# lavajuno/afskmodem

Measured on AMD Instinct MI355X. Metric: Msamples/s demodulated (batched 48 kHz streams) + decoded-byte match rate vs CPU ref, higher is better.
Workload: dtype int16

## Files before the change

### afskmodem_amd/batch.py

```python
from __future__ import annotations

import ctypes as C
import threading
import math
import os
from dataclasses import dataclass

import numpy as np

from . import _native

SAMPLE_RATE = _native.SAMPLE_RATE
SYNC_WINDOW = _native.SYNC_WINDOW


def validate_bit_frames(bit_frames) -> None:
    bf = np.atleast_1d(np.asarray(bit_frames))
    if np.any(bf <= 0) or np.any(SAMPLE_RATE % np.maximum(bf, 1) != 0) or np.any(bf % 2 != 0):
        raise Exception("Invalid baud rate.")
    if np.any(2 * bf >= SYNC_WINDOW):
        raise IndexError("list index out of range")
    if np.any(bf % 4 != 0):
        raise Exception("Comparing two waveforms of different lengths.")


_I32_MAX, _I32_MIN = 2 ** 31 - 1, -2 ** 31


def threshold_lt(t) -> int:
    t = float(t)
    if math.isnan(t):
        return _I32_MIN
    if math.isinf(t):
        return _I32_MAX if t > 0 else _I32_MIN
    return max(_I32_MIN, min(_I32_MAX, math.ceil(t)))


def threshold_gt(t) -> int:
    t = float(t)
    if math.isnan(t):
        return _I32_MAX
    if math.isinf(t):
        return _I32_MAX if t > 0 else _I32_MIN
    return max(_I32_MIN, min(_I32_MAX, math.floor(t)))


def out_stride_for(max_len: int, min_bit_frames: int) -> int:
    s = int(max_len // (14 * max(min_bit_frames, 4)) + 2 + 3) & ~3
    return s if s <= 192 else (s + 127) & ~127




@dataclass
class HostDemodResult:
    bytes: np.ndarray
    nbytes: np.ndarray
    nbits: np.ndarray
    clock_idx: np.ndarray
    term_frame: np.ndarray
    status: np.ndarray

    def payloads(self) -> list[bytes]:
        stride = self.bytes.shape[1]
        return [self.bytes[i, : min(int(n), stride)].tobytes() for i, n in enumerate(self.nbytes)]


def demod_host_arrays(arrays, bit_frames, amp_end_threshold: int = 14000) -> HostDemodResult:
    n = len(arrays)
    keep = [np.ascontiguousarray(a, dtype=np.int16).reshape(-1) for a in arrays]
    lens = np.array([a.size for a in keep], dtype=np.int32)
    bf = np.broadcast_to(np.asarray(bit_frames, dtype=np.int32), (n,)).copy()
    if n:
        validate_bit_frames(bf)
    stride = out_stride_for(int(lens.max()) if n else 0, int(bf.min()) if n else 4)
    res = HostDemodResult(np.zeros((n, stride), np.uint8), *(np.zeros(n, np.int32) for _ in range(5)))
    if n == 0:
        return res
    if n == 1:
        return demod_host_flat(keep[0], [0], lens, bf, amp_end_threshold, stride)
    ptrs = (C.c_void_p * n)(*[a.__array_interface__["data"][0] for a in keep])
    p = lambda a, t: a.ctypes.data_as(C.POINTER(t))
    _native.check(_native.lib().afsk_demod_streams_host(
        ptrs, p(lens, C.c_int32), p(bf, C.c_int32), threshold_lt(amp_end_threshold), n,
        p(res.bytes, C.c_uint8), stride, p(res.nbytes, C.c_int32), p(res.nbits, C.c_int32),
        p(res.clock_idx, C.c_int32), p(res.term_frame, C.c_int32), p(res.status, C.c_int32)))
    return res


def demod_host_flat(flat, stream_offset, stream_len, bit_frames,
                    amp_end_threshold: int = 14000, out_stride: int | None = None) -> HostDemodResult:
    flat = np.ascontiguousarray(flat, dtype=np.int16).reshape(-1)
    offs = np.ascontiguousarray(stream_offset, dtype=np.int64)
    lens = np.ascontiguousarray(stream_len, dtype=np.int32)
    n = offs.size
    bf = np.broadcast_to(np.asarray(bit_frames, dtype=np.int32), (n,)).copy()
    if n:
        validate_bit_frames(bf)
    stride = out_stride if out_stride is not None else out_stride_for(
        int(lens.max()) if n else 0, int(bf.min()) if n else 4)
    res = HostDemodResult(np.zeros((n, stride), np.uint8), *(np.zeros(n, np.int32) for _ in range(5)))
    if n == 0:
        return res
    total = flat.size
    if total == 0:
        flat = np.zeros(1, np.int16)
    p = lambda a, t: a.ctypes.data_as(C.POINTER(t))
    _native.check(_native.lib().afsk_demod_batch_host(
        p(flat, C.c_int16), total, p(offs, C.c_int64), p(lens, C.c_int32), p(bf, C.c_int32),
        threshold_lt(amp_end_threshold), n, p(res.bytes, C.c_uint8), stride, p(res.nbytes, C.c_int32),
        p(res.nbits, C.c_int32), p(res.clock_idx, C.c_int32), p(res.term_frame, C.c_int32),
        p(res.status, C.c_int32)))
    return res




def _torch():
    import torch
    return torch


@dataclass
class DemodResult:
    bytes: "object"
    nbytes: "object"
    nbits: "object"
    clock_idx: "object"
    term_frame: "object"
    status: "object"
    corrected: "object" = None
    margins: "object" = None

    def symbols_demodulated(self, bit_frames) -> "object":
        torch = _torch()
        bf = torch.as_tensor(bit_frames, device=self.nbits.device).to(torch.int64)
        found = (self.term_frame.to(torch.int64) - self.clock_idx.to(torch.int64)) // bf \
            + self.nbits.to(torch.int64)
        return found

    def cpu(self) -> HostDemodResult:
        return HostDemodResult(*(t.cpu().numpy() for t in
                                 (self.bytes, self.nbytes, self.nbits, self.clock_idx,
                                  self.term_frame, self.status)))

    def payloads(self) -> list[bytes]:
        return self.cpu().payloads()


def flat_layout(n_streams: int, out_stride: int):
    nb = (n_streams * out_stride + 3) & ~3
    offs = [0] + [nb + 4 * n_streams * k for k in range(5)]
    return offs, nb + 20 * n_streams


def views_of_flat(flat, n_streams: int, out_stride: int) -> "DemodResult":
    torch = _torch()
    offs, total = flat_layout(n_streams, out_stride)
    assert flat.numel() == total and flat.dtype == torch.uint8
    i32 = [flat[o: o + 4 * n_streams].view(torch.int32) for o in offs[1:]]
    res = DemodResult(flat[: n_streams * out_stride].view(n_streams, out_stride), *i32)
    res.flat = flat
    return res


def alloc_result(n_streams: int, out_stride: int, device) -> DemodResult:
    torch = _torch()
    _, total = flat_layout(n_streams, out_stride)
    return views_of_flat(torch.zeros(total, dtype=torch.uint8, device=device), n_streams, out_stride)


def uniform_layout(n_streams: int, stream_len: int, device):
    torch = _torch()
    off = torch.arange(n_streams, dtype=torch.int64, device=device) * int(stream_len)
    ln = torch.full((n_streams,), int(stream_len), dtype=torch.int32, device=device)
    return off, ln


def _as_device_i32(x, n, device):
    torch = _torch()
    if isinstance(x, torch.Tensor):
        return x.to(device=device, dtype=torch.int32).contiguous()
    arr = np.broadcast_to(np.asarray(x, dtype=np.int32), (n,)).copy()
    return torch.from_numpy(arr).to(device)


def _stream_ptr(stream, device=None):
    torch = _torch()
    s = stream if stream is not None else torch.cuda.current_stream(device)
    return C.c_void_p(s.cuda_stream)


def _same_device(dev, **tensors) -> None:
    for name, t in tensors.items():
        if t is not None and t.device != dev:
            raise ValueError(f"{name} is on {t.device}, samples on {dev}: all tensors of a launch must share one device")


def _order_after_current(stream, device) -> None:
    torch = _torch()
    if stream is not None:
        cur = torch.cuda.current_stream(device)
        if stream.cuda_stream != cur.cuda_stream:
            stream.wait_stream(cur)


def _uniform_bit_frames(bit_frames, n: int):
    if isinstance(bit_frames, (int, np.integer)):
        return int(bit_frames)
    if isinstance(bit_frames, (list, tuple, np.ndarray)):
        arr = np.asarray(bit_frames)
        if arr.ndim == 0:
            return int(arr)
        if arr.size not in (1, n):
            raise ValueError(f"bit_frames holds {arr.size} values for {n} streams (1 or {n} expected)")
        if arr.size and np.all(arr == arr.flat[0]):
            return int(arr.flat[0])
    return None


_PLAN_CACHE: "dict[tuple, GroupPlan]" = {}
_PLAN_CACHE_MAX = 8
_PLAN_CACHE_LOCK = threading.Lock()


def lengths_ragged(stream_len_host) -> bool:
    if stream_len_host is None:
        return False
    a = np.asarray(stream_len_host)
    return bool(a.size >= 8 and int(a.max()) > 0 and int(a.min()) * 4 < int(a.max()) * 3)


def _cached_plan(bit_frames, n: int, dev, stream_len_host=None) -> "GroupPlan":
    arr = np.asarray(bit_frames, dtype=np.int32)
    if arr.size not in (1, n):
        raise ValueError(f"bit_frames holds {arr.size} values for {n} streams (1 or {n} expected)")
    arr = np.ascontiguousarray(np.broadcast_to(arr.reshape(-1) if arr.ndim else arr, (n,)))
    lens = None
    if lengths_ragged(stream_len_host):
        lens = np.ascontiguousarray(np.asarray(stream_len_host, dtype=np.int32).reshape(-1))
        if lens.size != n:
            raise ValueError(f"stream_len_host holds {lens.size} values for {n} streams")
    key = (str(dev), n, hash(arr.tobytes()), None if lens is None else hash(lens.tobytes()))
    with _PLAN_CACHE_LOCK:
        plan = _PLAN_CACHE.pop(key, None)
        if plan is not None and np.array_equal(plan.bit_frames, arr) and (
                lens is None if plan.stream_len is None else (lens is not None and np.array_equal(plan.stream_len, lens))):
            _PLAN_CACHE[key] = plan
            return plan
    fresh = GroupPlan(arr, dev, stream_len=lens)
    with _PLAN_CACHE_LOCK:
        _PLAN_CACHE[key] = fresh
        while len(_PLAN_CACHE) > _PLAN_CACHE_MAX:
            _PLAN_CACHE.pop(next(iter(_PLAN_CACHE)))
    return fresh


class _NativePlan:
    _destroy: str

    def __init__(self, device):
        _native.require_device()
        _drain_parked_plans()
        self.device = _default_device(device)
        self._h = C.c_void_p()

    @property
    def handle(self):
        if not self._h:
            raise ValueError("the plan has been closed")
        return self._h

    def close(self) -> None:
        if self._h:
            getattr(_native.lib(), self._destroy)(self._h)
            self._h = C.c_void_p()

    def __del__(self):
        h = getattr(self, "_h", None)
        if not h:
            return
        self._h = None
        try:
            torch = _torch()
            if torch.cuda.is_current_stream_capturing():
                raise RuntimeError("capturing")
            torch.cuda.synchronize(self.device)
            getattr(_native.lib(), self._destroy)(h)
        except Exception:
            try:
                with _PARKED_LOCK:
                    _PARKED_PLANS.append((h, self.device, self._destroy))
            except Exception:
                pass


class GroupPlan(_NativePlan):
    _destroy = "afsk_group_plan_destroy"

    def __init__(self, bit_frames, device=None, stream_len=None):
        torch = _torch()
        super().__init__(device)
        self.bit_frames = np.ascontiguousarray(np.asarray(bit_frames, dtype=np.int32).reshape(-1))
        self.n = int(self.bit_frames.size)
        self.stream_len = None
        if stream_len is not None:
            self.stream_len = np.ascontiguousarray(np.asarray(stream_len, dtype=np.int32).reshape(-1))
            if self.stream_len.size != self.n:
                raise ValueError(f"stream_len holds {self.stream_len.size} values for {self.n} streams")
        i32 = C.POINTER(C.c_int32)
        with torch.cuda.device(self.device):
            _native.check(_native.lib().afsk_group_plan_create_ragged(
                self.bit_frames.ctypes.data_as(i32),
                None if self.stream_len is None else self.stream_len.ctypes.data_as(i32), self.n, C.byref(self._h)))

    def groups(self) -> list[tuple[int, int]]:
        ng, nn = C.c_int32(), C.c_int32()
        lib = _native.lib()
        _native.check(lib.afsk_group_plan_info(self.handle, C.byref(nn), C.byref(ng), None, None, 0))
        bf, cnt = (C.c_int32 * max(ng.value, 1))(), (C.c_int32 * max(ng.value, 1))()
        _native.check(lib.afsk_group_plan_info(self.handle, None, None, bf, cnt, ng.value))
        return [(int(bf[k]), int(cnt[k])) for k in range(ng.value)]


_PARKED_PLANS: list = []
_PARKED_LOCK = threading.Lock()


def _drain_parked_plans() -> None:
    if not _PARKED_PLANS:
        return
    torch = _torch()
    try:
        if torch.cuda.is_current_stream_capturing():
            return
    except Exception:
        return
    with _PARKED_LOCK:
        todo, _PARKED_PLANS[:] = list(_PARKED_PLANS), []
    for h, dev, destroy in todo:
        try:
            torch.cuda.synchronize(dev)
            getattr(_native.lib(), destroy)(h)
        except Exception:
            with _PARKED_LOCK:
                _PARKED_PLANS.append((h, dev, destroy))


def release_parked_plans() -> int:
    _drain_parked_plans()
    return len(_PARKED_PLANS)


def _check_index_tensors(dev, stream_offset, stream_len) -> None:
    torch = _torch()
    if stream_offset.dtype != torch.int64 or stream_len.dtype != torch.int32:
        raise TypeError("stream_offset must be int64 and stream_len int32")
    if not (stream_offset.is_cuda and stream_len.is_cuda):
        raise TypeError("stream_offset / stream_len must be CUDA tensors")
    _same_device(dev, stream_offset=stream_offset, stream_len=stream_len)
    if not (stream_offset.is_contiguous() and stream_len.is_contiguous()):
        raise ValueError("stream_offset / stream_len must be contiguous (the kernel reads them as plain arrays)")


def _prepare_outputs(out, out_stride, n: int, dev, diagnostics: bool, margin_stride):
    torch = _torch()
    fresh = False
    if out is None:
        if out_stride is None:
            raise ValueError("pass out= or out_stride=")
        out = alloc_result(n, int(out_stride), dev)
        fresh = True
    soft = (None, None, 0)
    if diagnostics:
        if out.corrected is None:
            out.corrected = torch.zeros(n, dtype=torch.int32, device=dev)
            fresh = True
        if out.margins is None:
            if margin_stride is None:
                raise ValueError("diagnostics=True needs margin_stride= (symbols per margins row)")
            out.margins = torch.zeros((n, int(margin_stride)), dtype=torch.int32, device=dev)
            fresh = True
        soft = (out.corrected.data_ptr(), out.margins.data_ptr(), int(out.margins.shape[1]))
    _same_device(dev, out_bytes=out.bytes, out_nbytes=out.nbytes, out_status=out.status)
    return out, fresh, (out.bytes.data_ptr(), int(out.bytes.shape[1]), out.nbytes.data_ptr(), out.nbits.data_ptr(),
                        out.clock_idx.data_ptr(), out.term_frame.data_ptr(), out.status.data_ptr(), *soft)


def demod_batch(samples, stream_offset, stream_len, bit_frames, amp_end_threshold: int = 14000,
                out: DemodResult | None = None, out_stride: int | None = None, stream=None,
                validate: bool = True, diagnostics: bool = False,
                margin_stride: int | None = None, entry: str = "auto", plan: "GroupPlan | None" = None,
                stream_len_host=None) -> DemodResult:
    torch = _torch()
    _native.require_device()
    if not (isinstance(samples, torch.Tensor) and samples.is_cuda and samples.dtype == torch.int16):
        raise TypeError("samples must be an int16 CUDA tensor (HBM resident)")
    if not samples.is_contiguous():
        raise ValueError("samples must be contiguous")
    if entry not in ("auto", "uniform", "grouped", "mixed"):
        raise ValueError("entry must be 'auto', 'uniform', 'grouped' or 'mixed'")
    n = int(stream_offset.numel())
    dev = samples.device
    if bit_frames is None and plan is None:
        raise ValueError("bit_frames=None needs plan= (the plan holds the batch's bit_frames)")
    if validate and bit_frames is not None and not isinstance(bit_frames, torch.Tensor):
        validate_bit_frames(bit_frames)
    _check_index_tensors(dev, stream_offset, stream_len)
    host_bf = isinstance(bit_frames, (int, np.integer, list, tuple, np.ndarray))
    if plan is not None:
        if entry not in ("auto", "grouped"):
            raise ValueError("plan= goes with entry='auto' or 'grouped'")
        if plan.n != n or plan.device != dev:
            raise ValueError(f"the plan covers {plan.n} streams on {plan.device}, the batch {n} on {dev}")
        entry = "grouped"
    ragged = plan is None and host_bf and entry in ("auto", "grouped") and lengths_ragged(stream_len_host)
    ubf = None if (entry in ("mixed", "grouped") or ragged) else _uniform_bit_frames(bit_frames, n)
    if entry == "uniform" and ubf is None:
        raise ValueError("entry='uniform' needs ONE bit_frames value (an int or an all-equal host sequence)")
    if entry == "grouped" and plan is None and not host_bf:
        raise ValueError("entry='grouped' needs host-side bit_frames (or plan=): a device tensor is never inspected")
    grouped = entry == "grouped" or ragged or (entry == "auto" and ubf is None and host_bf)
    out, fresh, outs = _prepare_outputs(out, out_stride, n, dev, diagnostics, margin_stride)
    amp = threshold_lt(amp_end_threshold)
    lib = _native.lib()
    with torch.cuda.device(dev):
        if fresh:
            _order_after_current(stream, dev)
        if ubf is not None:
            _native.check(lib.afsk_demod_batch_uniform(
                samples.data_ptr(), stream_offset.data_ptr(), stream_len.data_ptr(), ubf, amp, n, *outs,
                _stream_ptr(stream, dev)))
            return out
        if grouped:
            if plan is None:
                plan = _cached_plan(bit_frames, n, dev, stream_len_host if ragged else None)
            _native.check(lib.afsk_demod_batch_grouped(
                plan.handle, samples.data_ptr(), stream_offset.data_ptr(), stream_len.data_ptr(), amp, *outs,
                _stream_ptr(stream, dev)))
            out._plan_keepalive = plan
            return out
        bf = _as_device_i32(bit_frames, n, dev)
        _order_after_current(stream, dev)
        _native.check(lib.afsk_demod_batch_ex(
            samples.data_ptr(), stream_offset.data_ptr(), stream_len.data_ptr(), bf.data_ptr(), amp, n, *outs,
            _stream_ptr(stream, dev)))
    out._bf_keepalive = bf
    return out


VALID_BIT_FRAMES = tuple(bf for bf in range(4, SYNC_WINDOW // 2, 4) if SAMPLE_RATE % bf == 0)
assert len(VALID_BIT_FRAMES) == _native.DETECT_MAX_CANDIDATES


@dataclass
class HostRateResult:
    bit_frames: np.ndarray
    score: np.ndarray
    runner_up: np.ndarray
    clock_idx: np.ndarray
    scores: "np.ndarray | None"
    candidates: tuple

    def bauds(self) -> list:
        return [SAMPLE_RATE // int(bf) if bf > 0 else None for bf in self.bit_frames]


@dataclass
class RateResult:
    bit_frames: "object"
    score: "object"
    runner_up: "object"
    clock_idx: "object"
    scores: "object" = None
    candidates: tuple = ()

    def cpu(self) -> HostRateResult:
        h = lambda t: None if t is None else t.cpu().numpy()
        return HostRateResult(h(self.bit_frames), h(self.score), h(self.runner_up), h(self.clock_idx), h(self.scores),
                              self.candidates)

    def bauds(self) -> list:
        return self.cpu().bauds()


def check_candidates(candidates) -> tuple:
    if candidates is None:
        return VALID_BIT_FRAMES
    cands = tuple(int(c) for c in np.asarray(candidates).reshape(-1).tolist())
    if not 1 <= len(cands) <= _native.DETECT_MAX_CANDIDATES:
        raise ValueError(f"{len(cands)} candidates (1 ... {_native.DETECT_MAX_CANDIDATES} expected)")
    validate_bit_frames(cands)
    return cands


def detect_rates(samples, stream_offset, stream_len, candidates=None, out: RateResult | None = None, stream=None,
                 scores: bool = False) -> RateResult:
    torch = _torch()
    cands = check_candidates(candidates)
    _native.require_device()
    if not (isinstance(samples, torch.Tensor) and samples.is_cuda and samples.dtype == torch.int16):
        raise TypeError("samples must be an int16 CUDA tensor (HBM resident)")
    if not samples.is_contiguous():
        raise ValueError("samples must be contiguous")
    n = int(stream_offset.numel())
    dev = samples.device
    _check_index_tensors(dev, stream_offset, stream_len)
    if int(stream_len.numel()) != n:
        raise ValueError(f"{n} stream offsets for {int(stream_len.numel())} stream lengths")
    fresh = out is None
    if out is None:
        i32 = lambda *shape: torch.zeros(shape, dtype=torch.int32, device=dev)
        out = RateResult(i32(n), i32(n), i32(n), i32(n), i32(n, len(cands)) if scores else None, cands)
    else:
        want = {"bit_frames": (n,), "score": (n,), "runner_up": (n,), "clock_idx": (n,)}
        if scores or out.scores is not None:
            want["scores"] = (n, len(cands))
        for name, shape in want.items():
            t = getattr(out, name)
            if not (isinstance(t, torch.Tensor) and t.dtype == torch.int32 and tuple(t.shape) == shape
                    and t.is_contiguous()):
                raise ValueError(f"out.{name} must be a contiguous int32 tensor of shape {shape}")
        _same_device(dev, **{"out_" + name: getattr(out, name) for name in want})
        out.candidates = cands
    c_arr = (C.c_int32 * len(cands))(*cands)
    with torch.cuda.device(dev):
        if fresh:
            _order_after_current(stream, dev)
        _native.check(_native.lib().afsk_detect_rate_batch(
            samples.data_ptr(), stream_offset.data_ptr(), stream_len.data_ptr(), n, c_arr, len(cands),
            out.bit_frames.data_ptr(), out.score.data_ptr(), out.runner_up.data_ptr(), out.clock_idx.data_ptr(),
            None if out.scores is None else out.scores.data_ptr(), _stream_ptr(stream, dev)))
    return out


def _split_host_arrays(stream_len_host, bit_frames, segment_symbols):
    lens = np.ascontiguousarray(np.asarray(stream_len_host, dtype=np.int64).reshape(-1))
    n = int(lens.size)
    if n and (int(lens.min()) < 0 or int(lens.max()) > _native.MAX_STREAM_LEN):
        raise ValueError(f"stream lengths must lie in 0 ... {_native.MAX_STREAM_LEN}")
    bf = np.asarray(bit_frames)
    if bf.size not in (1, n) and not (n == 0 and bf.size == 0):
        raise ValueError(f"bit_frames holds {bf.size} values for {n} streams (1 or {n} expected)")
    bf = np.ascontiguousarray(np.broadcast_to(bf.reshape(-1) if bf.ndim else bf, (n,)).astype(np.int32))
    if n:
        validate_bit_frames(bf)
    segment_symbols = int(segment_symbols)
    if segment_symbols < 0 or segment_symbols % 64:
        raise ValueError("segment_symbols must be a multiple of 64 (0 = the default)")
    return lens.astype(np.int32), bf, segment_symbols


def split_scratch_bytes(stream_len_host, bit_frames, segment_symbols: int = 0) -> tuple[int, int]:
    lens, bf, seg = _split_host_arrays(stream_len_host, bit_frames, segment_symbols)
    i32 = C.POINTER(C.c_int32)
    nbytes, nseg = C.c_int64(), C.c_int32()
    _native.check(_native.lib().afsk_split_scratch_bytes(lens.ctypes.data_as(i32), bf.ctypes.data_as(i32), int(lens.size),
                                                         seg, C.byref(nbytes), C.byref(nseg)))
    return int(nbytes.value), int(nseg.value)


class SplitPlan(_NativePlan):
    _destroy = "afsk_split_plan_destroy"

    def __init__(self, stream_len_host, bit_frames, device=None, segment_symbols: int = 0):
        torch = _torch()
        lens, bf, seg = _split_host_arrays(stream_len_host, bit_frames, segment_symbols)
        super().__init__(device)
        self.stream_len = lens
        self.bit_frames = bf
        self.n = int(lens.size)
        self.segment_symbols = seg
        i32 = C.POINTER(C.c_int32)
        lib = _native.lib()
        with torch.cuda.device(self.device):
            _native.check(lib.afsk_split_plan_create(lens.ctypes.data_as(i32), bf.ctypes.data_as(i32), self.n, seg,
                                                     C.byref(self._h)))
            nseg, nbytes = C.c_int32(), C.c_int64()
            _native.check(lib.afsk_split_plan_info(self._h, None, C.byref(nseg), C.byref(nbytes)))
            self.n_segments = int(nseg.value)
            self.scratch_bytes = int(nbytes.value)
            self.scratch = torch.empty(max(self.scratch_bytes, 1), dtype=torch.uint8, device=self.device)


def demod_batch_split(samples, stream_offset, stream_len, plan: SplitPlan, amp_end_threshold: int = 14000,
                      out: DemodResult | None = None, out_stride: int | None = None, stream=None,
                      diagnostics: bool = False, margin_stride: int | None = None) -> DemodResult:
    torch = _torch()
    if not isinstance(plan, SplitPlan):
        raise TypeError("plan must be a SplitPlan")
    if not (isinstance(samples, torch.Tensor) and samples.dtype == torch.int16):
        raise TypeError("samples must be an int16 CUDA tensor (HBM resident)")
    if not (isinstance(stream_offset, torch.Tensor) and isinstance(stream_len, torch.Tensor)):
        raise TypeError("stream_offset / stream_len must be CUDA tensors")
    if stream_offset.dtype != torch.int64 or stream_len.dtype != torch.int32:
        raise TypeError("stream_offset must be int64 and stream_len int32")
    n = int(stream_offset.numel())
    if plan.n != n or int(stream_len.numel()) != n:
        raise ValueError(f"the plan covers {plan.n} streams, the batch {n}")
    if out is None and out_stride is None:
        raise ValueError("pass out= or out_stride=")
    if diagnostics and (out is None or out.margins is None) and margin_stride is None:
        raise ValueError("diagnostics=True needs margin_stride= (symbols per margins row)")
    _native.require_device()
    if not samples.is_cuda:
        raise TypeError("samples must be an int16 CUDA tensor (HBM resident)")
    if not samples.is_contiguous():
        raise ValueError("samples must be contiguous")
    dev = samples.device
    _check_index_tensors(dev, stream_offset, stream_len)
    if plan.device != dev:
        raise ValueError(f"the plan was built on {plan.device}, the batch lives on {dev}")
    out, fresh, outs = _prepare_outputs(out, out_stride, n, dev, diagnostics, margin_stride)
    with torch.cuda.device(dev):
        if fresh:
            _order_after_current(stream, dev)
        _native.check(_native.lib().afsk_demod_batch_split(
            plan.handle, samples.data_ptr(), stream_offset.data_ptr(), stream_len.data_ptr(),
            threshold_lt(amp_end_threshold), plan.scratch.data_ptr(), *outs, _stream_ptr(stream, dev)))
    out._plan_keepalive = plan
    return out


@dataclass
class GateResult:
    n_bursts: "object"
    burst_start: "object"
    burst_len: "object"
    open_end: "object"
    block_amp: "object"
    slot_offset: "object" = None
    slot_len: "object" = None

    def burst_streams(self, stream_offset):
        torch = _torch()
        nb = self.burst_start.shape[1]
        mask = torch.arange(nb, device=self.n_bursts.device)[None, :] < self.n_bursts[:, None]
        owner, k = torch.nonzero(mask, as_tuple=True)
        off = stream_offset[owner] + self.burst_start[owner, k].to(torch.int64)
        return owner, off.contiguous(), self.burst_len[owner, k].contiguous()

    def burst_slots(self, stream_offset):
        if self.slot_len is not None:
            return self.slot_offset.reshape(-1), self.slot_len.reshape(-1)
        torch = _torch()
        nb = self.burst_start.shape[1]
        mask = torch.arange(nb, device=self.n_bursts.device)[None, :] < self.n_bursts[:, None]
        off = torch.where(mask, stream_offset[:, None] + self.burst_start.to(torch.int64), 0)
        ln = torch.where(mask, self.burst_len, 0)
        return off.reshape(-1).contiguous(), ln.reshape(-1).contiguous()


def gate_batch(samples, stream_offset, stream_len, max_stream_len: int,
               amp_start_threshold: int = 18000, amp_end_threshold: int = 14000,
               max_bursts: int = 16, stream=None, slots: bool = True) -> GateResult:
    torch = _torch()
    _native.require_device()
    if not (isinstance(samples, torch.Tensor) and samples.is_cuda and samples.dtype == torch.int16
            and samples.is_contiguous()):
        raise TypeError("samples must be a contiguous int16 CUDA tensor")
    if stream_offset.dtype != torch.int64 or stream_len.dtype != torch.int32:
        raise TypeError("stream_offset must be int64 and stream_len int32")
    n = int(stream_offset.numel())
    dev = samples.device
    _same_device(dev, stream_offset=stream_offset, stream_len=stream_len)
    max_blocks = int(max_stream_len) // 2048
    i32 = lambda *shape: torch.zeros(shape, dtype=torch.int32, device=dev)
    with torch.cuda.device(dev):
        res = GateResult(i32(n), i32(n, max(max_bursts, 1)), i32(n, max(max_bursts, 1)), i32(n),
                         i32(n, max(max_blocks, 1)))
        if slots and max_bursts > 0:
            res.slot_offset = torch.zeros((n, int(max_bursts)), dtype=torch.int64, device=dev)
            res.slot_len = i32(n, int(max_bursts))
        _order_after_current(stream, dev)
        args = (samples.data_ptr(), stream_offset.data_ptr(), stream_len.data_ptr(), int(max_stream_len),
                threshold_gt(amp_start_threshold), threshold_lt(amp_end_threshold), n, int(max_bursts),
                res.block_amp.data_ptr(), res.n_bursts.data_ptr(), res.burst_start.data_ptr(),
                res.burst_len.data_ptr(), res.open_end.data_ptr())
        if res.slot_len is not None:
            _native.check(_native.lib().afsk_gate_batch_slots(*args, res.slot_offset.data_ptr(), res.slot_len.data_ptr(),
                                                              _stream_ptr(stream, dev)))
        else:
            _native.check(_native.lib().afsk_gate_batch(*args, _stream_ptr(stream, dev)))
    return res


def _default_device(device):
    torch = _torch()
    return torch.device("cuda", torch.cuda.current_device()) if device is None else torch.device(device)


def upload_streams(arrays, device=None):
    torch = _torch()
    _native.require_device()
    device = _default_device(device)
    lens = np.array([len(a) for a in arrays], dtype=np.int32)
    offs = np.zeros(len(arrays), dtype=np.int64)
    if len(arrays) > 1:
        offs[1:] = np.cumsum(lens[:-1], dtype=np.int64)
    flat = (np.concatenate([np.ascontiguousarray(a, dtype=np.int16) for a in arrays])
            if len(arrays) else np.zeros(0, np.int16))
    if flat.size == 0:
        flat = np.zeros(1, np.int16)
    t = lambda a: torch.from_numpy(a).to(device)
    return t(flat), t(offs), t(lens), int(lens.max()) if len(arrays) else 0


def read_wav_frames(filename: str) -> np.ndarray:
    import wave
    with wave.open(filename, "rb") as f:
        raw = f.readframes(f.getnframes())
    return np.frombuffer(raw, dtype="<i2", count=len(raw) // 2)


def _c_names(filenames):
    import sys
    strs = [f if type(f) is str else os.fsdecode(os.fspath(f)) for f in filenames]
    if not strs:
        return (b"", None), (C.c_char_p * 0)()
    blob = ("\0".join(strs) + "\0").encode(sys.getfilesystemencoding(), sys.getfilesystemencodeerrors())
    a = np.frombuffer(blob, np.uint8)
    ends = np.flatnonzero(a == 0)
    if ends.size != len(strs):
        raise ValueError("embedded null byte")
    ptrs = np.empty(len(strs), np.uint64)
    ptrs[0] = 0
    ptrs[1:] = ends[:-1] + 1
    ptrs += np.uint64(a.ctypes.data)
    return (blob, ptrs), C.cast(ptrs.ctypes.data, C.POINTER(C.c_char_p))


def _wav_probe_c(arr, n):
    off = np.zeros(n, np.int64)
    nbytes = np.zeros(n, np.int64)
    status = np.zeros(n, np.int32)
    if n:
        p = lambda a, t: a.ctypes.data_as(C.POINTER(t))
        _native.check(_native.lib().afsk_wav_probe(arr, n, p(off, C.c_int64), p(nbytes, C.c_int64),
                                                   p(status, C.c_int32)))
    return off, nbytes, status


def wav_probe(filenames):
    names = list(filenames)
    keep, arr = _c_names(names)
    res = _wav_probe_c(arr, len(names))
    del keep
    return res


def load_wav_batch(filenames, device=None):
    torch = _torch()
    _native.require_device()
    device = _default_device(device)
    names = list(filenames)
    if not names:
        return upload_streams([], device)
    n = len(names)
    enc, arr = _c_names(names)
    lib = _native.lib()
    p64 = lambda a: a.ctypes.data_as(C.POINTER(C.c_int64))
    sizes = np.zeros(n, np.int64)
    _native.check(lib.afsk_file_sizes(arr, n, p64(sizes)))
    slot = np.minimum(((np.maximum(sizes, 0) // 2) + 7) & ~np.int64(7), np.int64(_native.MAX_STREAM_LEN & ~7))
    offs = np.zeros(n, np.int64)
    offs[1:] = np.cumsum(slot[:-1])
    total = int(offs[-1] + slot[-1])
    samples = torch.empty(max(total, 1), dtype=torch.int16, device=device)
    if total == 0:
        samples.zero_()
    d_off = np.zeros(n, np.int64)
    d_bytes = np.zeros(n, np.int64)
    status = np.zeros(n, np.int32)
    torch.cuda.current_stream(samples.device).synchronize()
    with torch.cuda.device(samples.device):
        _native.check(lib.afsk_wav_ingest(arr, n, p64(offs), p64(slot), samples.data_ptr(), int(samples.numel()),
                                          p64(d_off), p64(d_bytes), status.ctypes.data_as(C.POINTER(C.c_int32))))
    lens = (d_bytes // 2).astype(np.int64)
    bad = np.nonzero(status != _native.WAV_OK)[0]
    if bad.size:
        lens[bad] = 0
        late = []
        for i in bad:
            fr = read_wav_frames(names[int(i)])
            lens[i] = len(fr)
            if len(fr) <= int(slot[i]):
                if len(fr):
                    samples[int(offs[i]): int(offs[i]) + len(fr)] = torch.from_numpy(np.ascontiguousarray(fr)).to(device)
            else:
                late.append((int(i), fr))
        if late:
            extra = torch.from_numpy(np.concatenate([np.ascontiguousarray(fr) for _, fr in late])).to(device)
            pos = total
            samples = torch.cat([samples[:total], extra])
            for i, fr in late:
                offs[i] = pos
                pos += len(fr)
    if int(lens.max()) > _native.MAX_STREAM_LEN:
        raise ValueError("a stream longer than AFSK_MAX_STREAM_LEN samples")
    t = lambda a: torch.from_numpy(a).to(device)
    return samples, t(offs), t(lens.astype(np.int32)), int(lens.max())


def save_wav_batch(samples, stream_offset, stream_len, filenames) -> np.ndarray:
    torch = _torch()
    _native.require_device()
    if not (isinstance(samples, torch.Tensor) and samples.is_cuda and samples.dtype == torch.int16
            and samples.is_contiguous()):
        raise TypeError("samples must be a contiguous int16 CUDA tensor")
    names = list(filenames)
    n = len(names)
    host = lambda a, dt: np.ascontiguousarray(a.cpu().numpy() if isinstance(a, torch.Tensor) else a, dtype=dt)
    offs, lens = host(stream_offset, np.int64), host(stream_len, np.int32)
    if offs.size != n or lens.size != n:
        raise ValueError(f"{n} file names for {offs.size} offsets / {lens.size} lengths")
    status = np.zeros(n, np.int32)
    if n == 0:
        return status
    if int((offs + lens).max()) > samples.numel():
        raise ValueError("a stream reaches beyond the sample buffer")
    keep, arr = _c_names(names)
    torch.cuda.current_stream(samples.device).synchronize()
    with torch.cuda.device(samples.device):
        _native.check(_native.lib().afsk_wav_egress(arr, n, samples.data_ptr(), offs.ctypes.data_as(C.POINTER(C.c_int64)),
                                                    lens.ctypes.data_as(C.POINTER(C.c_int32)),
                                                    status.ctypes.data_as(C.POINTER(C.c_int32))))
    del keep
    return status


def modulate_batch(payload, payload_len, bit_frames, ts_cycles, stream_offset, stream_len,
                   max_stream_len: int, samples, wav_quirk: bool = True, stream=None) -> None:
    torch = _torch()
    _native.require_device()
    n = int(stream_offset.numel())
    for t, dt in ((payload, torch.uint8), (payload_len, torch.int32), (bit_frames, torch.int32),
                  (ts_cycles, torch.int32), (stream_offset, torch.int64),
                  (stream_len, torch.int32), (samples, torch.int16)):
        if not (isinstance(t, torch.Tensor) and t.is_cuda and t.dtype == dt and t.is_contiguous()):
            raise TypeError("modulate_batch wants contiguous CUDA tensors of the documented dtypes")
    dev = samples.device
    _same_device(dev, payload=payload, payload_len=payload_len, bit_frames=bit_frames, ts_cycles=ts_cycles,
                 stream_offset=stream_offset, stream_len=stream_len)
    with torch.cuda.device(dev):
        _native.check(_native.lib().afsk_modulate_batch(
            payload.data_ptr(), int(payload.shape[1]), payload_len.data_ptr(), bit_frames.data_ptr(),
            ts_cycles.data_ptr(), stream_offset.data_ptr(), stream_len.data_ptr(),
            int(max_stream_len), n, 1 if wav_quirk else 0, samples.data_ptr(), _stream_ptr(stream, dev)))


def add_noise_batch(samples, stream_offset, stream_len, max_stream_len: int, scale_q24, seed: int,
                    stream_idx_base: int = 0, stream=None) -> None:
    torch = _torch()
    _native.require_device()
    n = int(stream_offset.numel())
    dev = samples.device
    _same_device(dev, stream_offset=stream_offset, stream_len=stream_len)
    with torch.cuda.device(dev):
        sc = _as_device_i32(scale_q24, n, dev)
        _order_after_current(stream, dev)
        _native.check(_native.lib().afsk_add_noise_batch(
            samples.data_ptr(), stream_offset.data_ptr(), stream_len.data_ptr(), int(max_stream_len),
            sc.data_ptr(), n, int(seed) & 0xFFFFFFFF, int(stream_idx_base) & 0xFFFFFFFF,
            _stream_ptr(stream, dev)))
        (stream if stream is not None else torch.cuda.current_stream(dev)).synchronize()
```

### afskmodem_amd/csrc/afsk_gate.hip

```cpp
#include "afsk_kernels.h"
#include "afsk_capi_internal.h"

namespace afsk {

constexpr int kListenBlock = 2048;

typedef uint32_t vec16 __attribute__((ext_vector_type(4), aligned(2)));

__device__ __forceinline__ int block_abs_sum(const vec16 (&v)[4]) {
    uint32_t acc = 0;
#pragma unroll
    for (int j = 0; j < 4; j++)
#pragma unroll
        for (int k = 0; k < 4; k++)
            acc = __builtin_amdgcn_sad_u16(v[j][k] ^ 0x80008000u, 0x80008000u, acc);
    int t = (int)acc;
    t += __builtin_amdgcn_update_dpp(0, t, 0x111, 0xf, 0xf, true);
    t += __builtin_amdgcn_update_dpp(0, t, 0x112, 0xf, 0xf, true);
    t += __builtin_amdgcn_update_dpp(0, t, 0x114, 0xf, 0xf, true);
    t += __builtin_amdgcn_update_dpp(0, t, 0x118, 0xf, 0xf, true);
    t += __builtin_amdgcn_update_dpp(0, t, 0x142, 0xa, 0xf, false);
    t += __builtin_amdgcn_update_dpp(0, t, 0x143, 0xc, 0xf, false);
    return t;
}

__global__ __launch_bounds__(256) void block_amp_kernel(GateArgs a) {
    const int lane = threadIdx.x & 63;
    const int64_t w = (int64_t)xcd_block((int)blockIdx.x, (int)gridDim.x) * 4 + (threadIdx.x >> 6);
    const int s = (int)(w / a.max_blocks);
    if (s >= a.n_streams) return;
    const int b = (int)(w - (int64_t)s * a.max_blocks);
    const int32_t len = a.stream_len[s];
    if ((uint32_t)len > (uint32_t)a.max_len) return;
    const int32_t nb = len / kListenBlock;
    if (b >= nb) return;
    const int16_t* src = a.samples + a.stream_offset[s] + (int64_t)b * kListenBlock;
    vec16 v[4];
#pragma unroll
    for (int j = 0; j < 4; j++)
        v[j] = __builtin_nontemporal_load(reinterpret_cast<const vec16*>(src + 512 * j + 8 * lane));
    const int t = block_abs_sum(v);
    if (lane == 63) a.block_amp[(int64_t)s * a.max_blocks + b] = (int32_t)((uint32_t)t >> 11);
}

__global__ __launch_bounds__(256) void gate_scan_kernel(GateArgs a) {
    const int s = blockIdx.x * blockDim.x + threadIdx.x;
    if (s >= a.n_streams) return;
    const int32_t len = a.stream_len[s];
    if ((uint32_t)len > (uint32_t)a.max_len) {
        a.out_n_bursts[s] = -1;
        a.out_open_end[s] = 0;
        if (a.out_slot_len)
            for (int k = 0; k < a.max_bursts; k++) {
                a.out_slot_offset[(int64_t)s * a.max_bursts + k] = 0;
                a.out_slot_len[(int64_t)s * a.max_bursts + k] = 0;
            }
        return;
    }
    const int32_t nb = len / kListenBlock;
    const int32_t* amp = a.block_amp + (int64_t)s * a.max_blocks;
    int32_t* bs = a.out_burst_start + (int64_t)s * a.max_bursts;
    int32_t* bl = a.out_burst_len + (int64_t)s * a.max_bursts;
    int n = 0, open_end = 0;
    int mode = 0;
    int start = 0;
    for (int b = 0; b < nb && n < a.max_bursts; b++) {
        if (mode == 0) { mode = 1; continue; }
        const int32_t v = amp[b];
        if (mode == 1) {
            if (v > a.amp_start) { start = b; mode = 2; }
        } else if (v < a.amp_end) {
            bs[n] = start * kListenBlock;
            bl[n] = (b - start + 1) * kListenBlock;
            n++;
            mode = 0;
        }
    }
    if (mode == 2 && n < a.max_bursts) {
        bs[n] = start * kListenBlock;
        bl[n] = (nb - start) * kListenBlock;
        n++;
        open_end = 1;
    }
    a.out_n_bursts[s] = n;
    a.out_open_end[s] = open_end;
    if (a.out_slot_len) {
        const int64_t base = a.stream_offset[s];
        for (int k = 0; k < a.max_bursts; k++) {
            a.out_slot_offset[(int64_t)s * a.max_bursts + k] = k < n ? base + bs[k] : 0;
            a.out_slot_len[(int64_t)s * a.max_bursts + k] = k < n ? bl[k] : 0;
        }
    }
}

hipError_t launch_gate(const GateArgs& a, hipStream_t stream) {
    if (a.n_streams <= 0) return hipSuccess;
    if (a.max_blocks > 0) {
        const int64_t waves = (int64_t)a.n_streams * a.max_blocks;
        const int64_t blocks = (waves + 3) / 4;
        if (blocks > 0x7fffffffll) return hipErrorInvalidValue;
        hipLaunchKernelGGL(block_amp_kernel, dim3((uint32_t)blocks), dim3(256), 0, stream, a);
        hipError_t e = hipGetLastError();
        if (e != hipSuccess) return e;
    }
    hipLaunchKernelGGL(gate_scan_kernel, dim3((a.n_streams + 255) / 256), dim3(256), 0, stream, a);
    return hipGetLastError();
}

__global__ __launch_bounds__(256) void clear_i32_kernel(int32_t* out, int64_t n) {
    const int64_t i = (int64_t)blockIdx.x * 256 + threadIdx.x;
    if (i < n) out[i] = 0;
}

hipError_t launch_clear_i32(int32_t* out, int64_t n, hipStream_t stream) {
    if (n <= 0) return hipSuccess;
    const int64_t blocks = (n + 255) / 256;
    if (blocks > 0x7fffffffll) return hipErrorInvalidValue;
    hipLaunchKernelGGL(clear_i32_kernel, dim3((uint32_t)blocks), dim3(256), 0, stream, out, n);
    return hipGetLastError();
}

}

#include "afsk_split.hip"
#include "afsk_live.hip"
#include "afsk_live_stream.hip"
#include "afsk_live_tap.hip"
#include "afsk_live_auto.hip"
#include "afsk_live_push.hip"
#include "afsk_live_pack.hip"
#include "afsk_detect.hip"
```

Before: 3.791 million.

## Use wave-per-stream ballot gate scan and drop output zero-fill allocations

Adds a gate scan kernel that assigns one 64-lane wave per stream. It finds burst starts and ends with ballot masks and ctz instead of a serial per-thread loop, and spreads the output stores across lanes. The Python side now allocates outputs with empty instead of zeros, and the kernels write every element, including zeros for unused blocks and bursts, which removes the memset launches. The wave path runs when the stream count is at or below an env-configurable threshold; otherwise the old per-thread scan is used, now also clearing unused slots. Correctness depends on the kernels covering every output element.

```diff
diff --git a/afskmodem_amd/batch.py b/afskmodem_amd/batch.py
--- a/afskmodem_amd/batch.py
+++ b/afskmodem_amd/batch.py
@@ -665,12 +665,12 @@
     dev = samples.device
     _same_device(dev, stream_offset=stream_offset, stream_len=stream_len)
     max_blocks = int(max_stream_len) // 2048
-    i32 = lambda *shape: torch.zeros(shape, dtype=torch.int32, device=dev)
+    i32 = lambda *shape: torch.empty(shape, dtype=torch.int32, device=dev)
+    col = lambda k: i32(n, k) if k > 0 else torch.zeros((n, 1), dtype=torch.int32, device=dev)
     with torch.cuda.device(dev):
-        res = GateResult(i32(n), i32(n, max(max_bursts, 1)), i32(n, max(max_bursts, 1)), i32(n),
-                         i32(n, max(max_blocks, 1)))
+        res = GateResult(i32(n), col(int(max_bursts)), col(int(max_bursts)), i32(n), col(max_blocks))
         if slots and max_bursts > 0:
-            res.slot_offset = torch.zeros((n, int(max_bursts)), dtype=torch.int64, device=dev)
+            res.slot_offset = torch.empty((n, int(max_bursts)), dtype=torch.int64, device=dev)
             res.slot_len = i32(n, int(max_bursts))
         _order_after_current(stream, dev)
         args = (samples.data_ptr(), stream_offset.data_ptr(), stream_len.data_ptr(), int(max_stream_len),
diff --git a/afskmodem_amd/csrc/afsk_gate.hip b/afskmodem_amd/csrc/afsk_gate.hip
--- a/afskmodem_amd/csrc/afsk_gate.hip
+++ b/afskmodem_amd/csrc/afsk_gate.hip
@@ -1,3 +1,4 @@
+#include <cstdlib>
 #include "afsk_kernels.h"
 #include "afsk_capi_internal.h"
 
@@ -31,33 +32,95 @@
     if (s >= a.n_streams) return;
     const int b = (int)(w - (int64_t)s * a.max_blocks);
     const int32_t len = a.stream_len[s];
-    if ((uint32_t)len > (uint32_t)a.max_len) return;
-    const int32_t nb = len / kListenBlock;
-    if (b >= nb) return;
+    if ((uint32_t)len > (uint32_t)a.max_len || b >= len / kListenBlock) {
+        if (lane == 63) a.block_amp[w] = 0;
+        return;
+    }
     const int16_t* src = a.samples + a.stream_offset[s] + (int64_t)b * kListenBlock;
     vec16 v[4];
 #pragma unroll
     for (int j = 0; j < 4; j++)
         v[j] = __builtin_nontemporal_load(reinterpret_cast<const vec16*>(src + 512 * j + 8 * lane));
     const int t = block_abs_sum(v);
-    if (lane == 63) a.block_amp[(int64_t)s * a.max_blocks + b] = (int32_t)((uint32_t)t >> 11);
+    if (lane == 63) a.block_amp[w] = (int32_t)((uint32_t)t >> 11);
+}
+
+__device__ __forceinline__ void gate_scan_wave(const GateArgs& a, int s, const int32_t* amp) {
+    const int lane = threadIdx.x & 63;
+    const int32_t first = lane < a.max_blocks ? amp[lane] : 0;
+    const int32_t len = a.stream_len[s];
+    const bool refused = (uint32_t)len > (uint32_t)a.max_len;
+    const int32_t nb = refused ? 0 : len / kListenBlock;
+    const int64_t row = (int64_t)s * a.max_bursts;
+    const int64_t base = a.out_slot_len ? a.stream_offset[s] : 0;
+    int n = 0, open_end = 0;
+    int mode = 0, start = 0;
+    int32_t rec_start = 0, rec_len = 0;
+    auto store = [&](int k0) {
+        const int k = k0 + lane;
+        if (k >= a.max_bursts) return;
+        const bool used = k < n;
+        a.out_burst_start[row + k] = used ? rec_start : 0;
+        a.out_burst_len[row + k] = used ? rec_len : 0;
+        if (a.out_slot_len) {
+            a.out_slot_offset[row + k] = used ? base + rec_start : 0;
+            a.out_slot_len[row + k] = used ? rec_len : 0;
+        }
+    };
+    auto record = [&](int from, int blocks) {
+        if (lane == (n & 63)) { rec_start = from * kListenBlock; rec_len = blocks * kListenBlock; }
+        n++;
+        if ((n & 63) == 0) store(n - 64);
+    };
+    for (int p0 = 0; p0 < nb && n < a.max_bursts; p0 += 64) {
+        const int cnt = min(64, nb - p0);
+        const int32_t v = p0 == 0 ? first : lane < cnt ? amp[p0 + lane] : 0;
+        const uint64_t ms = __ballot(lane < cnt && v > a.amp_start);
+        const uint64_t me = __ballot(lane < cnt && v < a.amp_end);
+        int c = 0;
+        while (n < a.max_bursts) {
+            if (mode == 0) {
+                if (c >= cnt) break;
+                c++;
+                mode = 1;
+            }
+            if (mode == 1) {
+                const uint64_t m = c < 64 ? ms >> c << c : 0;
+                if (!m) break;
+                c = __builtin_ctzll(m);
+                start = p0 + c++;
+                mode = 2;
+            }
+            const uint64_t m = c < 64 ? me >> c << c : 0;
+            if (!m) break;
+            c = __builtin_ctzll(m) + 1;
+            record(start, p0 + c - start);
+            mode = 0;
+        }
+    }
+    if (mode == 2 && n < a.max_bursts) {
+        record(start, nb - start);
+        open_end = 1;
+    }
+    for (int k0 = n & ~63; k0 < a.max_bursts; k0 += 64) store(k0);
+    if (lane == 0) {
+        a.out_n_bursts[s] = refused ? -1 : n;
+        a.out_open_end[s] = open_end;
+    }
+}
+
+__global__ __launch_bounds__(256) void gate_scan_wave_kernel(GateArgs a) {
+    const int64_t s = (int64_t)blockIdx.x * 4 + __builtin_amdgcn_readfirstlane(threadIdx.x >> 6);
+    if (s >= a.n_streams) return;
+    gate_scan_wave(a, (int)s, a.block_amp + s * a.max_blocks);
 }
 
 __global__ __launch_bounds__(256) void gate_scan_kernel(GateArgs a) {
     const int s = blockIdx.x * blockDim.x + threadIdx.x;
     if (s >= a.n_streams) return;
     const int32_t len = a.stream_len[s];
-    if ((uint32_t)len > (uint32_t)a.max_len) {
-        a.out_n_bursts[s] = -1;
-        a.out_open_end[s] = 0;
-        if (a.out_slot_len)
-            for (int k = 0; k < a.max_bursts; k++) {
-                a.out_slot_offset[(int64_t)s * a.max_bursts + k] = 0;
-                a.out_slot_len[(int64_t)s * a.max_bursts + k] = 0;
-            }
-        return;
-    }
-    const int32_t nb = len / kListenBlock;
+    const bool refused = (uint32_t)len > (uint32_t)a.max_len;
+    const int32_t nb = refused ? 0 : len / kListenBlock;
     const int32_t* amp = a.block_amp + (int64_t)s * a.max_blocks;
     int32_t* bs = a.out_burst_start + (int64_t)s * a.max_bursts;
     int32_t* bl = a.out_burst_len + (int64_t)s * a.max_bursts;
@@ -82,15 +145,23 @@
         n++;
         open_end = 1;
     }
-    a.out_n_bursts[s] = n;
+    a.out_n_bursts[s] = refused ? -1 : n;
     a.out_open_end[s] = open_end;
-    if (a.out_slot_len) {
-        const int64_t base = a.stream_offset[s];
-        for (int k = 0; k < a.max_bursts; k++) {
+    const int64_t base = a.out_slot_len ? a.stream_offset[s] : 0;
+    for (int k = 0; k < a.max_bursts; k++) {
+        if (k >= n) bs[k] = bl[k] = 0;
+        if (a.out_slot_len) {
             a.out_slot_offset[(int64_t)s * a.max_bursts + k] = k < n ? base + bs[k] : 0;
             a.out_slot_len[(int64_t)s * a.max_bursts + k] = k < n ? bl[k] : 0;
         }
     }
+}
+
+constexpr int32_t kWaveScanMaxCaptures = 8192;
+
+static int32_t wave_scan_max_captures() {
+    const char* e = std::getenv("AFSK_GATE_WAVE_SCAN_MAX");
+    return (e && *e) ? (int32_t)std::atol(e) : kWaveScanMaxCaptures;
 }
 
 hipError_t launch_gate(const GateArgs& a, hipStream_t stream) {
@@ -103,7 +174,10 @@
         hipError_t e = hipGetLastError();
         if (e != hipSuccess) return e;
     }
-    hipLaunchKernelGGL(gate_scan_kernel, dim3((a.n_streams + 255) / 256), dim3(256), 0, stream, a);
+    if (a.n_streams <= wave_scan_max_captures())
+        hipLaunchKernelGGL(gate_scan_wave_kernel, dim3((uint32_t)(((int64_t)a.n_streams + 3) / 4)), dim3(256), 0, stream, a);
+    else
+        hipLaunchKernelGGL(gate_scan_kernel, dim3((a.n_streams + 255) / 256), dim3(256), 0, stream, a);
     return hipGetLastError();
 }
 
```

New measurement: 3.791 million (median of 2 runs). About the same (+0.0%).
